# Geryyy/sspp

Hardware: AMD Instinct MI355X
Metric: candidate paths scored/sec (7-DoF, 128 waypts) at 1/2/4/8 MI355X; HBM %peak (higher is better)
Workload: dtype f64; 1 GPU; robocrane SamplingPathPlanner7 (block_green free joint), sigma 0.08; candidates_per_gpu=4096, waypoints=128, init_points=10, degree=3, dof=7, sampler=fp64, pair_order=hit, waypoint_order=hit, sampled_pairs=4, cylinder_box=False, capsule=False, scan=fp32-filtered, split=True, split_lost=0, split_handoffs=0, streams=4

## Files before the change

### include/sspp_hip.h

```cpp
#ifndef SSPP_HIP_H
#define SSPP_HIP_H
#include <stddef.h>
#include <stdint.h>

#ifdef __cplusplus
extern "C" {
#endif

#define SSPP_OK 0
#define SSPP_E_INVAL (-1)
#define SSPP_E_HIP (-2)
#define SSPP_E_SCENE (-3)
#define SSPP_E_NOMEM (-4)
#define SSPP_E_UNSUPPORTED (-5)
#define SSPP_E_IO (-6)
#define SSPP_E_INCOMPLETE (-7)

#define SSPP_GEOM_PLANE 0
#define SSPP_GEOM_SPHERE 2
#define SSPP_GEOM_CAPSULE 3
#define SSPP_GEOM_CYLINDER 5
#define SSPP_GEOM_BOX 6
#define SSPP_GEOM_MESH 7

// ... 111 lines not shown
                              double* d_vias_out , sspp_best* d_best,
                              void* stream);
int sspp_job_tsp_score_vias(sspp_job* job, const double* d_vias ,
                            int64_t first_id, int64_t B, double* d_L, double* d_Cnf,
                            double* d_Cwf, uint8_t* d_status, double* d_cost, sspp_best* d_best,
                            void* stream);
int sspp_job_info(const sspp_job* job, int* lanes_per_candidate, int* candidates_per_block,
                  int* block_threads, size_t* lds_bytes);
void sspp_job_free(sspp_job* job);

#define SSPP_OPT_SHAPE_NT 1
#define SSPP_OPT_SHAPE_G1 2
#define SSPP_OPT_ORDER 3
#define SSPP_OPT_TSP_FORM 4
#define SSPP_OPT_TSP_GENERIC 5
#define SSPP_OPT_SAMPLER 6
#define SSPP_OPT_LAST_NT 7
#define SSPP_OPT_LAST_G1 8
#define SSPP_OPT_WP_ORDER 9
#define SSPP_OPT_PREPASS_US 10
#define SSPP_OPT_NPAIRS 11
#define SSPP_OPT_CYLBOX 12
#define SSPP_OPT_F32 13
#define SSPP_OPT_LAST_F32 14
#define SSPP_OPT_CREATE_US 15
#define SSPP_OPT_PREPASS_STATE 16
#define SSPP_OPT_SPLIT 17
#define SSPP_OPT_LAST_SPLIT 18
#define SSPP_OPT_SPLIT_LINGER_US 20
#define SSPP_OPT_SPLIT_DROP 21
#define SSPP_OPT_SPLIT_HANDOFFS 22
#define SSPP_OPT_SPLIT_LOST 23
#define SSPP_OPT_CAPSULE 24
#define SSPP_OPT_TSP_REP 19
int sspp_job_set_option(sspp_job* job, int key, int64_t value);
int sspp_job_get_option(const sspp_job* job, int key, int64_t* value);

typedef struct sspp_ces sspp_ces;
typedef struct sspp_ces_config {
    int samples;
    int checks;
    int total_points;
    double w_collision, elite_fraction, inc, dec;
    double sigma_floor, var_beta, mean_lr, stddev_min, stddev_max;
    double z_min;
    double dist_z_min;
    double sigma0;
    const double* lo;
    const double* hi;
    double floor_z_min, floor_margin, floor_scale;
    uint64_t seed;
} sspp_ces_config;
typedef struct sspp_ces_info {
    int n_vias, n_slots, slots_per_rank, world, elite_capacity;
    int64_t iteration;
} sspp_ces_info;
typedef struct sspp_ces_state {
    int n_fixed;
    int n_candidates;
    int n_success, n_elite, has_best;
    int64_t best_slot;
    double best_cost;
    int64_t iteration;
} sspp_ces_state;
typedef struct sspp_ces_buffers {
    double *L, *C_nf, *C_wf, *cost;
// ... 78 lines not shown
```

### sspp_amd/_lib.py

```python
from __future__ import annotations

import ctypes as C
import os
import re

_HERE = os.path.dirname(os.path.abspath(__file__))
PRODUCT_LIB_PATH = os.path.join(_HERE, "lib", "libsspp_hip.so")
LIB_PATH = os.environ.get("SSPP_LIB_PATH") or PRODUCT_LIB_PATH
HEADER_PATH = os.path.join(os.path.dirname(_HERE), "include", "sspp_hip.h")

SSPP_OK = 0
SSPP_E_INCOMPLETE = -7
MODE_QPOS = 0
MODE_BODY = 1


class SsppError(RuntimeError):
    pass


class ModelView(C.Structure):
    _fields_ = [
        ("nbody", C.c_int), ("body_parent", C.POINTER(C.c_int32)),
        ("body_jnt_type", C.POINTER(C.c_int32)), ("body_qpos_adr", C.POINTER(C.c_int32)),
# ... 110 lines not shown
    "sspp_job_update_sspp": (C.c_int, [_vp, _d, C.c_double, _d, C.c_uint64, _vp]),
    "sspp_planner_create": (C.c_int, [_vp, _i, C.POINTER(_vp)]),
    "sspp_planner_plan": (C.c_int, [_vp, _d, _d, C.c_double, _d, _i, _i, _i, C.c_uint64, _i64, _d,
                                    C.POINTER(_i64), C.POINTER(_i64), _d, _d, C.POINTER(Best)]),
    "sspp_planner_score": (C.c_int, [_vp, _d, _i, _d, _i64, _i, _i, _i, _d, C.POINTER(C.c_uint8),
                                     C.POINTER(Best)]),
    "sspp_planner_free": (None, [_vp]),
    "sspp_planner_get_option": (C.c_int, [_vp, _i, C.POINTER(_i64)]),
    "sspp_ces_create": (C.c_int, [_vp, C.POINTER(CesConfig), _i, C.POINTER(_vp)]),
    "sspp_ces_get_info": (C.c_int, [_vp, C.POINTER(CesInfo)]),
    "sspp_ces_begin": (C.c_int, [_vp, _d, _d, _i, _vp]),
    "sspp_ces_eval": (C.c_int, [_vp, _i, _vp]),
    "sspp_ces_update": (C.c_int, [_vp, _vp]),
    "sspp_ces_plan": (C.c_int, [_vp, _d, _d, _i, _i, _vp]),
    "sspp_ces_plan_group": (C.c_int, [_vp, _i, _d, _d, _i, _i, _vp]),
    "sspp_ces_get_buffers": (C.c_int, [_vp, C.POINTER(CesBuffers)]),
    "sspp_ces_read": (C.c_int, [_vp, C.POINTER(CesState), _vp, _vp, _vp, _vp, _vp, _vp, _vp, _vp,
                                _vp, _vp]),
    "sspp_ces_set_state": (C.c_int, [_vp, _vp, _vp, _vp, _i]),
    "sspp_ces_pack": (C.c_int, [_vp, _i, _vp, _vp]),
    "sspp_ces_unpack": (C.c_int, [_vp, _vp, _vp]),
    "sspp_ces_free": (None, [_vp]),
    "sspp_job_set_option": (C.c_int, [_vp, _i, _i64]),
    "sspp_job_get_option": (C.c_int, [_vp, _i, C.POINTER(_i64)]),
    "sspp_ces_set_option": (C.c_int, [_vp, _i, _i64]),
}

OPT_SHAPE_NT, OPT_SHAPE_G1, OPT_ORDER, OPT_TSP_FORM, OPT_TSP_GENERIC = 1, 2, 3, 4, 5
OPT_SAMPLER, OPT_LAST_NT, OPT_LAST_G1, OPT_WP_ORDER, OPT_PREPASS_US, OPT_NPAIRS = 6, 7, 8, 9, 10, 11
OPT_CYLBOX, OPT_F32, OPT_LAST_F32, OPT_CREATE_US, OPT_PREPASS_STATE = 12, 13, 14, 15, 16
OPT_SPLIT, OPT_LAST_SPLIT, OPT_TSP_REP = 17, 18, 19
OPT_SPLIT_LINGER_US, OPT_SPLIT_DROP, OPT_SPLIT_HANDOFFS, OPT_SPLIT_LOST = 20, 21, 22, 23
OPT_CAPSULE = 24
OPT_CES_FUSED = 101


def declared_symbols(header=HEADER_PATH):
    txt = open(header).read()
    txt = re.sub(r"/\*.*?\*/", "", txt, flags=re.S)
    return sorted(set(re.findall(r"\b(sspp_[a-z_0-9]+)\s*\(", txt)))


_lib = None
build_warning = None


def check_revision(L, path, variant):
    from ._stamp import source_hash
    tree = source_hash()
    f = getattr(L, "sspp_build_id", None)
    built = None
    if f is not None:
        f.restype, f.argtypes = C.c_char_p, []
        built = (f() or b"").decode(errors="replace")
    if tree is None or built == tree:
        return None
    what = ("built from sources %s" % built) if built else "no source stamp (sspp_build_id)"
    msg = "%s: %s, but the tree's sources are %s" % (path, what, tree)
    if variant:
        raise SsppError("stale variant library " + msg +
                        " (rebuild it: bash tools/build_variant.sh NAME FLAGS)")
    import warnings
    warnings.warn("libsspp_hip.so does not match its sources: " + msg + " (run `make`)", RuntimeWarning)
    return msg


# ... 26 lines not shown
```

### sspp_amd/csrc/sspp_kern.h

```cpp
#pragma once
#include <hip/hip_runtime.h>

#include <algorithm>
#include <atomic>
#include <cstdlib>
#include <cmath>
#include <cstring>
#include <string>
#include <thread>
#include <vector>

#include "model.h"
#ifndef SSPP_TSP_REP_FORMS
#define SSPP_TSP_REP_FORMS (1 << 3)
#endif
#ifdef SSPP_TSP_STATS
__device__ unsigned long long g_tsp_stats[16];
#define TSP_STAT(i, c) do { const unsigned long long m_ = __ballot(c), a_ = __ballot(1);                  \
        if (__lane_id() == __builtin_ctzll(a_) && m_) atomicAdd(&g_tsp_stats[i], (unsigned long long)__popcll(m_)); } while (0)
#else
#define TSP_STAT(i, c) do { } while (0)
#endif
#ifdef SSPP_C2F_STATS
__device__ unsigned long long g_c2f_stats[16];
#define SSPP_CB_STAT(i) atomicAdd(&g_c2f_stats[i], 1ull)
#endif
#ifdef SSPP_WG_TIMING
__device__ unsigned long long g_wg_t[1 << 18];
__device__ unsigned long long g_wg_ph[8 << 16];
#define WG_PH(k) do { if (threadIdx.x == 0 && blockIdx.x < (1 << 16)) g_wg_ph[8 * blockIdx.x + (k)] = clock64(); } while (0)
__device__ unsigned long long g_p2_t[8 << 12];
__device__ unsigned long long g_p2_w[8 << 13];
#else
#define WG_PH(k) do { } while (0)
#endif
#include "sspp_device.h"
#include "sspp_filter.h"
#include "sspp_logtab.h"

using namespace sspd;

namespace sspk {

constexpr int kBlock = 256;
#ifndef SSPP_SCORE_WAVES_PER_EU
#define SSPP_SCORE_WAVES_PER_EU 4
#endif
constexpr int kMaxMovers = 2;
constexpr int kMaxSteps = 64;

constexpr int kTableCylBox = 1, kTableCapsule = 2;
__host__ __device__ inline int table_bits(int tg, int to) {
    return (((tg == 5 && to == 6) || (tg == 6 && to == 5)) ? kTableCylBox : 0) |
           (sspd::pair_has_capsule(tg, to) ? kTableCapsule : 0);
}

struct KScene {
    int npairs;
    int onegeom;
    int static_block;
    double static_cost;
    int cylbox;
    int upright;
    int cbup;
};
// ... 748 lines not shown
#define SSPP_QUEUE_ACQUIRE() do { } while (0)
#endif
#ifndef SSPP_SPLIT_PRIO
#define SSPP_SPLIT_PRIO 1
#endif
#ifndef SSPP_PRIO_ALL
#define SSPP_PRIO_ALL 0
#endif
#ifndef SSPP_SPLIT_PRIO_CONSUMER
#define SSPP_SPLIT_PRIO_CONSUMER 0
#endif
#ifndef SSPP_QUEUE_WAITERS
#define SSPP_QUEUE_WAITERS 4
#endif
#ifndef SSPP_LINGER_SLEEP
#define SSPP_LINGER_SLEEP 16
#endif
constexpr int kSurvShards = 64;
struct SurvShard {
    unsigned count;
    unsigned taken;
    unsigned pushed;
    unsigned served;
    unsigned pad[28];
};
struct SurvQ {
    SurvShard shard[kSurvShards];
    unsigned nlist;
    unsigned lost;
    unsigned norphan;
    unsigned pad1;
    unsigned long long handoffs;
    unsigned long long lost_total;
    unsigned pad2[24];
    unsigned arrive_sh[8][32];
    unsigned arrive_top[32];
    unsigned long long bestbits[kMaxSteps];
    unsigned count_feas[kMaxSteps];
};
__host__ __device__ inline unsigned long long surv_word(int step, long long lc, bool defer) {
    return (1ull << 63) | ((unsigned long long)defer << 62) | ((unsigned long long)(unsigned)step << 32) |
           (unsigned long long)(unsigned)lc;
}
struct SurvBest {
    unsigned long long bits, id, step, pad;
};
struct SurvPtrs {
    SurvQ* hdr;
    unsigned long long* rec;
    double* ctrl;
    float* ctrl32;
    SurvBest* res;
    unsigned* orphan;
#ifdef SSPP_DEBUG_PROGRESS
    unsigned* beacon;
#endif
    long long cap;
    int shard_cap;
};

struct SsppC2F {
    KScene sc;
    int has_scene;
    int sampler;
    int p, n, W;
    double sigma;
    unsigned long long seed;
    long long first_id, B;
    int g1, cpw, cpb;
    int npts, n1;
    int lpc;
    int nblk_step;
    long long step_stride;
    int arc_all;
    int r0, r1;
    int nt;
    int lds;
    int ctrl_feas;
    int f32;
    float feps, fplim;
    int split;
    int nsteps;
    int drop_orphans;
    unsigned long long linger;
};

#ifdef SSPP_C2F_STATS
#define C2F_STAT(i, v) do { const unsigned long long v_ = (v); if ((threadIdx.x & 63) == 0 && v_) atomicAdd(&g_c2f_stats[i], v_); } while (0)
#else
#define C2F_STAT(i, v) do { } while (0)
#endif

__device__ __forceinline__ int crow(int mine, int fix, int r0, int r1, int j, int D) {
    return (j >= r0 && j < r1) ? mine + (j - r0) * D : fix + j * D;
}
template <int D, int P>
__device__ __forceinline__ void eval_split(const double* sm, int mine, int fix, int r0, int r1,
                                           const double (&Nr)[P + 1], int span, double* q) {
    int o[P + 1];
#pragma unroll
    for (int r = 0; r <= P; ++r) o[r] = crow(mine, fix, r0, r1, span - P + r, D);
#pragma unroll
    for (int d = 0; d < D; ++d) {
        double acc = Nr[0] * sm[o[0] + d];
#pragma unroll
// ... 402 lines not shown
#pragma unroll
                for (int d = 0; d < D; ++d) qa[d] = __shfl_up(qb[d], 1, 64);
                if (lane == 0) eval_split_g<D, P>(smem, o_own, o_fix, r0, r1, atab + jj * P1, aspan[jj], qa);
                if (jc < nch) acc = acc + dist_nd<D>(qa, qb);
            }
            acc = wave_sum(acc);
            if (lane == 0) s_vsum[vw] = acc;
        }
        SSPP_BEACON(23, slot, 0);
        __syncthreads();
        total = s_vsum[0];
        for (int w = 1; w < nvw; ++w) total = total + s_vsum[w];
    }
    if (tid == 0) {
        const long long c = (long long)step * a.B + lc;
        arc[c] = total;
        feasible[c] = (unsigned char)feas;
        if (with_best) {
            if (feas && total < INFINITY) {
                const unsigned long long bits = (unsigned long long)__double_as_longlong(total);
                const unsigned long long seen =
                    __hip_atomic_fetch_min(q.hdr->bestbits + step, bits, __ATOMIC_RELAXED, __HIP_MEMORY_SCOPE_AGENT);
                if (bits <= seen) {
                    const unsigned k = __hip_atomic_fetch_add(&q.hdr->nlist, 1u, __ATOMIC_RELAXED, __HIP_MEMORY_SCOPE_AGENT);
                    __hip_atomic_store(&q.res[k].bits, bits, __ATOMIC_RELAXED, __HIP_MEMORY_SCOPE_AGENT);
                    __hip_atomic_store(&q.res[k].id, (unsigned long long)(a.first_id + step * a.step_stride + lc),
                                       __ATOMIC_RELAXED, __HIP_MEMORY_SCOPE_AGENT);
                    __hip_atomic_store(&q.res[k].step, (unsigned long long)step, __ATOMIC_RELAXED, __HIP_MEMORY_SCOPE_AGENT);
                }
            }
            if (feas) __hip_atomic_fetch_add(q.hdr->count_feas + step, 1u, __ATOMIC_RELAXED, __HIP_MEMORY_SCOPE_AGENT);
        }
#ifdef SSPP_WG_TIMING
        unsigned long long* t = g_p2_w + 8 * (slot & ((8u << 10) - 1u));
        t[0] = w_t0; t[1] = wall_clock64(); t[2] = w_np; t[3] = w_nf; t[4] = feas;
        t[5] = c1 - c0; t[6] = clock64() - c1; t[7] = blockIdx.x;
#endif
    }
    (void)slot;
    SSPP_BEACON(24, slot, 0);
    __syncthreads();
}

#ifndef SSPP_C2F_WAVES_PER_EU
#define SSPP_C2F_WAVES_PER_EU 5
#endif
#ifndef SSPP_C2F_WAVES_PER_EU_WIDE
#define SSPP_C2F_WAVES_PER_EU_WIDE 4
#endif
#ifndef SSPP_ABLATE
#define SSPP_ABLATE 0
#endif
template <int D, int NM, int P, bool ONEGEOM, int NT, bool CBX, bool SPLIT = false>
#ifndef SSPP_C2F_FIVE_MAX
#define SSPP_C2F_FIVE_MAX 128
#endif
#ifndef SSPP_C2F_GP_NT
#define SSPP_C2F_GP_NT 256
#endif
__global__ __launch_bounds__(NT, (NT <= SSPP_C2F_FIVE_MAX && ONEGEOM) ? SSPP_C2F_WAVES_PER_EU : SSPP_C2F_WAVES_PER_EU_WIDE) void k_sspp_c2f(
    SsppC2F a, SceneT T, const double* __restrict__ otab, const float* __restrict__ otab32,
    const int* __restrict__ ospan,
    const double* __restrict__ atab, const int* __restrict__ aspan,
    const double* __restrict__ init_ctrl, const double* __restrict__ limits,
    const double* __restrict__ ctrl_in, double* __restrict__ ctrl_out, double* __restrict__ arc,
    unsigned char* __restrict__ feasible, BlockBest* __restrict__ part, ArgminSync* sync, sspp_best* best,
    SurvPtrs q) {
    extern __shared__ __attribute__((aligned(16))) double smem[];
    constexpr int P1 = P + 1;
// ... 102 lines not shown
    {
        const bool valid = in_grp && g < nvalid;
        bool ghit = false, dfr = false;
        if (collide_on) {
            const bool live = valid && l < a.n1 && !a.sc.static_block && !(ABL & 16);
            const int own = o_own + (valid ? g : 0) * nrd;
            if (f32) {
                float q32[D];
                eval_split32<D, P>(s_f32, own, o_fix, r0, r1, N32_p1, span_p1, q32);
                unsigned long long amb;
                ghit = scan_pairs32<D, NM, ONEGEOM>(q32, live, ~0ull, ~0ull, gbits, a.sc, TT, a.feps, a.fplim, amb);
                const bool need = live && !ghit && amb != 0ull;
                C2F_STAT(11, __popcll(__ballot(need)));
                if (__ballot(need) != 0ull) {
                    double q[D];
                    eval_split_g<D, P>(smem, own, o_fix, r0, r1, otab + row_p1 * P1, span_p1, q);
                    ghit = scan_pairs<D, NM, ONEGEOM, CBX ? 1 : 0>(q, need, amb, wave_or64(need ? amb : 0ull), gbits, nullptr,
                                                      a.sc, TT, dfr) || ghit;
                }
            } else {
                double q[D];
                eval_split_g<D, P>(smem, own, o_fix, r0, r1, otab + row_p1 * P1, span_p1, q);
                ghit = scan_pairs<D, NM, ONEGEOM, CBX ? 1 : 0>(q, live, ~0ull, ~0ull, gbits, nullptr, a.sc, TT, dfr);
            }
        }
        const bool gdef = (__ballot(dfr) & gbits) != 0ull;
        if (in_grp && l == 0 && g < cpb) {
            s_feas[g] = valid && !ghit && !(collide_on && a.sc.static_block);
            s_defer[g] = gdef;
        }
    }
    __syncthreads();
    WG_PH(3);
    if constexpr ((SPLIT || SSPP_PRIO_ALL) && SSPP_SPLIT_PRIO) __builtin_amdgcn_s_setprio(SSPP_SPLIT_PRIO_CONSUMER);
    if constexpr (SPLIT) {
        static_assert(NM == 1 && ONEGEOM && !CBX, "split launches: single-geom movers without cylinder-box pairs");
        int tid_s = threadIdx.x;
        asm volatile("" : "+v"(tid_s));
        const int tid = tid_s;
        SSPP_BEACON(3, 0, 0);
        SSPP_BEACON_T(1);
        if (tid < 64) {
            const bool f = tid < nvalid && s_feas[tid] != 0;
            const unsigned long long m = __ballot(f);
            unsigned base = 0;
            if (tid == 0 && m)
                base = __hip_atomic_fetch_add(&q.hdr->shard[blockIdx.x % kSurvShards].count, (unsigned)__popcll(m),
                                              __ATOMIC_RELAXED, __HIP_MEMORY_SCOPE_AGENT);
            base = (unsigned)__shfl((int)base, 0, 64) + (unsigned)((blockIdx.x % kSurvShards) * q.shard_cap);
            if (tid < cpb) s_surv[tid] = f ? (int)(base + __popcll(m & ((1ull << tid) - 1ull))) : -1;
        }
        __syncthreads();
        for (int e = tid; e < nvalid * nrd; e += NT) {
            const int sl = e / nrd, r = e - sl * nrd, slot = s_surv[sl];
            if (slot >= 0) {
                const long long o = (long long)slot * nrd + r;
                __hip_atomic_store((unsigned long long*)q.ctrl + o,
                                   (unsigned long long)__double_as_longlong(smem[o_own + sl * nrd + r]),
                                   __ATOMIC_RELAXED, __HIP_MEMORY_SCOPE_AGENT);
                __hip_atomic_store((unsigned*)q.ctrl32 + o, __float_as_uint(s_f32[o_own + sl * nrd + r]),
                                   __ATOMIC_RELAXED, __HIP_MEMORY_SCOPE_AGENT);
            }
        }
        asm volatile("s_waitcnt vmcnt(0)" ::: "memory");
        __syncthreads();
        if (tid < nvalid) {
            const int slot = s_surv[tid];
            if (slot >= 0) {
                __hip_atomic_store(q.rec + slot, surv_word(step, cand0 + tid, s_defer[tid] != 0), SSPP_QUEUE_RELEASE_ORDER,
                                   __HIP_MEMORY_SCOPE_AGENT);
            } else {
                arc[tid + cand0] = INFINITY;
                feasible[tid + cand0] = 0;
            }
        }
        asm volatile("s_waitcnt vmcnt(0)" ::: "memory");
        __syncthreads();
        if (tid == 0)
            __hip_atomic_fetch_add(&q.hdr->shard[blockIdx.x % kSurvShards].pushed, 1u, __ATOMIC_RELAXED,
                                   __HIP_MEMORY_SCOPE_AGENT);
        SSPP_BEACON(4, __popcll(__ballot(tid < nvalid && s_surv[tid] >= 0)), __smid());
        SSPP_BEACON_T(2);
        const unsigned nb_all = gridDim.x, shs = blockIdx.x % kSurvShards;
        const unsigned nwg_s = (nb_all - shs + kSurvShards - 1) / kSurvShards;
        SurvShard* const sh = q.hdr->shard + shs;
        int* s_ctl = s_surv;
        int* s_last = s_surv + cpb;
        bool last = false;
        unsigned ko = 0, no = 0;
        unsigned handed = 0;
#ifdef SSPP_DEBUG_PROGRESS
        unsigned nfin = 0;
#endif
        for (;;) {
            if (tid == 0) {
                unsigned t = ~0u;
                unsigned long long w = 0ull;
                if (!last) {
                    const unsigned tk0 = __hip_atomic_load(&sh->taken, __ATOMIC_RELAXED, __HIP_MEMORY_SCOPE_AGENT);
                    const unsigned ct0 = __hip_atomic_load(&sh->count, __ATOMIC_RELAXED, __HIP_MEMORY_SCOPE_AGENT);
                    if ((int)(tk0 - ct0) < SSPP_QUEUE_WAITERS) {
                        t = __hip_atomic_fetch_add(&sh->taken, 1u, __ATOMIC_RELAXED, __HIP_MEMORY_SCOPE_AGENT);
                        SSPP_BEACON(5, t, ct0);
                        const unsigned long long w0 = wall_clock64();
                        for (;;) {
                            if (t < __hip_atomic_load(&sh->count, __ATOMIC_RELAXED, __HIP_MEMORY_SCOPE_AGENT)) break;
                            if (__hip_atomic_load(&sh->pushed, __ATOMIC_RELAXED, __HIP_MEMORY_SCOPE_AGENT) >= nwg_s &&
                                __hip_atomic_load(&sh->count, __ATOMIC_RELAXED, __HIP_MEMORY_SCOPE_AGENT) <= t) {
                                t = ~0u;
                                break;
                            }
                            if (wall_clock64() - w0 >= a.linger) {
                                const unsigned k = __hip_atomic_fetch_add(&q.hdr->norphan, 1u, __ATOMIC_RELAXED,
                                                                          __HIP_MEMORY_SCOPE_AGENT);
                                __hip_atomic_store(q.orphan + k, t + shs * (unsigned)q.shard_cap, __ATOMIC_RELAXED,
                                                   __HIP_MEMORY_SCOPE_AGENT);
                                handed = 1;
                                t = ~0u;
                                break;
                            }
                            __builtin_amdgcn_s_sleep(SSPP_LINGER_SLEEP);
                        }
                    }
                    if (t != ~0u) {
                        t += shs * (unsigned)q.shard_cap;
                        SSPP_BEACON(6, t, 0);
                        const unsigned long long w1 = wall_clock64();
                        while ((w = __hip_atomic_load(q.rec + t, __ATOMIC_RELAXED, __HIP_MEMORY_SCOPE_AGENT)) == 0ull) {
                            if (wall_clock64() - w1 >= a.linger) break;
                            __builtin_amdgcn_s_sleep(1);
                        }
// ... 47 lines not shown
                const unsigned nblk = gridDim.x;
                const int shd = blockIdx.x & 7, nsh = nblk < 8 ? (int)nblk : 8;
                if (tid == 0) {
                    asm volatile("s_waitcnt vmcnt(0)" ::: "memory");
                    const unsigned shard_n = (nblk - shd + 7) >> 3;
                    const unsigned prev = __hip_atomic_fetch_add(&q.hdr->arrive_sh[shd][0], 1u + (handed << 16),
                                                                 __ATOMIC_RELAXED, __HIP_MEMORY_SCOPE_AGENT);
                    int lst = 0;
                    if ((prev & 0xFFFFu) == shard_n - 1) {
                        const unsigned sho = (prev >> 16) + handed;
                        const unsigned pt = __hip_atomic_fetch_add(&q.hdr->arrive_top[0], 1u + (sho << 16),
                                                                   __ATOMIC_RELAXED, __HIP_MEMORY_SCOPE_AGENT);
                        lst = (pt & 0xFFFFu) == (unsigned)nsh - 1;
                        if (lst) {
                            SSPP_QUEUE_ACQUIRE();
                            no = (pt >> 16) + sho;
                        }
                    }
                    s_last[0] = lst;
                    s_last[1] = (int)no;
                }
                __syncthreads();
                const int lst = __builtin_amdgcn_readfirstlane(s_last[0]);
                SSPP_BEACON(9 + lst, no, 0);
                if (lst) SSPP_BEACON_E(0);
                if (!lst) return;
                if (__builtin_amdgcn_readfirstlane(s_last[1]) == 0) break;
                last = true;
                continue;
            }
            const unsigned long long w = ((unsigned long long)(unsigned)__builtin_amdgcn_readfirstlane(s_ctl[2]) << 32) |
                                         (unsigned)__builtin_amdgcn_readfirstlane(s_ctl[3]);
            SSPP_BEACON(7, t, (unsigned)w);
            surv_load_rows<NT>(q, t, nrd, smem, s_f32, o_own);
            __syncthreads();
            surv_finish<D, NM, P, ONEGEOM, NT>(a, TT, otab, otab32, ospan, atab, aspan, smem, s_f32, o_fix, o_own,
                                               s_ctl, s_vsum, w, t, arc_base, feas_base, best_base != nullptr, q);
            if (tid == 0)
                __hip_atomic_fetch_add(&q.hdr->shard[t / (unsigned)q.shard_cap].served, 1u, __ATOMIC_RELAXED,
                                       __HIP_MEMORY_SCOPE_AGENT);
#ifdef SSPP_DEBUG_PROGRESS
            if (tid == 0 && q.beacon) q.beacon[8 * blockIdx.x + 3] = ++nfin;
#endif
        }
#ifdef SSPP_WG_TIMING
        const unsigned long long t_ep = wall_clock64();
#endif
        asm volatile("s_waitcnt vmcnt(0)" ::: "memory");
        __syncthreads();
        SSPP_BEACON(12, no, 0);
        SSPP_BEACON_E(1);
        int tid_e = threadIdx.x;
        asm volatile("" : "+v"(tid_e));
        const int tid_ep = tid_e;
        unsigned long long* s_bits = (unsigned long long*)smem;
        unsigned long long* s_id = s_bits + kMaxSteps;
        unsigned* s_cnt = (unsigned*)(s_id + kMaxSteps);
        unsigned* s_lost = s_cnt + kMaxSteps;
        const int nsteps = a.nsteps;
        const unsigned nl = __hip_atomic_load(&q.hdr->nlist, __ATOMIC_RELAXED, __HIP_MEMORY_SCOPE_AGENT);
        unsigned c_sh = 0, sv_sh = 0;
        if (tid_ep < kSurvShards) {
            c_sh = __hip_atomic_load(&q.hdr->shard[tid_ep].count, __ATOMIC_RELAXED, __HIP_MEMORY_SCOPE_AGENT);
            sv_sh = __hip_atomic_load(&q.hdr->shard[tid_ep].served, __ATOMIC_RELAXED, __HIP_MEMORY_SCOPE_AGENT);
        }
        unsigned long long rb = 0ull, rid = 0ull, rst = 0ull;
        if (best_base) {
            rb = __hip_atomic_load(&q.res[tid_ep].bits, __ATOMIC_RELAXED, __HIP_MEMORY_SCOPE_AGENT);
            rid = __hip_atomic_load(&q.res[tid_ep].id, __ATOMIC_RELAXED, __HIP_MEMORY_SCOPE_AGENT);
            rst = __hip_atomic_load(&q.res[tid_ep].step, __ATOMIC_RELAXED, __HIP_MEMORY_SCOPE_AGENT);
        }
        for (int e = tid_ep; e < nsteps; e += NT) {
            s_bits[e] = __hip_atomic_load(q.hdr->bestbits + e, __ATOMIC_RELAXED, __HIP_MEMORY_SCOPE_AGENT);
            s_cnt[e] = __hip_atomic_load(q.hdr->count_feas + e, __ATOMIC_RELAXED, __HIP_MEMORY_SCOPE_AGENT);
            s_id[e] = ~0ull;
        }
        const unsigned short_sh = c_sh > sv_sh ? c_sh - sv_sh : 0u;
        if (tid_ep < 64) {
            const unsigned tot = (unsigned)wave_sum_u32((int)short_sh);
            if (tid_ep == 0) s_lost[0] = tot;
        }
        __syncthreads();
        const unsigned lost = (unsigned)__builtin_amdgcn_readfirstlane((int)s_lost[0]);
        SSPP_BEACON_E(2);
        if (short_sh)
            for (unsigned e = 0; e < c_sh; ++e)
                __hip_atomic_store(q.rec + (unsigned)tid_ep * (unsigned)q.shard_cap + e, 0ull, __ATOMIC_RELAXED,
                                   __HIP_MEMORY_SCOPE_AGENT);
        if (tid_ep == 0) {
            if (lost) __hip_atomic_fetch_add(&q.hdr->lost_total, (unsigned long long)lost, __ATOMIC_RELAXED,
                                             __HIP_MEMORY_SCOPE_AGENT);
            if (no) __hip_atomic_fetch_add(&q.hdr->handoffs, (unsigned long long)no, __ATOMIC_RELAXED,
                                           __HIP_MEMORY_SCOPE_AGENT);
        }
        if (best_base) {
            if ((unsigned)tid_ep < nl && rb == s_bits[rst]) atomicMin(s_id + rst, rid);
            for (unsigned i = tid_ep + NT; i < nl; i += NT) {
                const unsigned long long bits = __hip_atomic_load(&q.res[i].bits, __ATOMIC_RELAXED, __HIP_MEMORY_SCOPE_AGENT);
                const unsigned long long id = __hip_atomic_load(&q.res[i].id, __ATOMIC_RELAXED, __HIP_MEMORY_SCOPE_AGENT);
                const int st = (int)__hip_atomic_load(&q.res[i].step, __ATOMIC_RELAXED, __HIP_MEMORY_SCOPE_AGENT);
                if (bits == s_bits[st]) atomicMin(s_id + st, id);
            }
        }
        __syncthreads();
        SSPP_BEACON_E(3);
        for (int e = tid_ep; e < nsteps; e += NT) {
            if (best_base) {
                const bool has = s_id[e] != ~0ull;
                best_base[e].cost = has ? __longlong_as_double((long long)s_bits[e]) : INFINITY;
                best_base[e].index = has ? (long long)s_id[e] : -1;
                best_base[e].count = s_cnt[e];
                best_base[e].reserved = lost;
            }
// ... 905 lines not shown
    double* d_pp_term = nullptr;
    unsigned* d_pp_arrive = nullptr;
    int64_t pp_cap = 0;
    unsigned char* h_pin = nullptr;
    size_t h_pin_bytes = 0;
    hipEvent_t upd_ev = nullptr;
    bool upd_pending = false;
    double start[4], end[4], lo[4], hi[4];
    double z_min = 0, w_col = 1, floor_z_min = 0, floor_margin = 0.01, floor_scale = 10;
    std::thread prepass_thread;
    std::atomic<int> prepass_state{0};
    std::vector<int> pre_wps;
    std::vector<DPair> pre_pairs, pre_pairs_s;
    double pre_ms = 0.0;
    int pre_gen = 0;
    int tables_gen = 0;
    hipStream_t pre_stream = nullptr;
    hipEvent_t pre_ev = nullptr;
    unsigned long long* d_hits = nullptr;
    unsigned long long* h_hits = nullptr;
    DPair* d_census_pairs = nullptr;
    std::vector<void*> retired;
    double create_ms = 0.0;
    int opt_split = 1;
    int last_split = 0;
    SurvQ* d_sq_hdr = nullptr;
    unsigned long long* d_sq_rec = nullptr;
    double* d_sq_ctrl = nullptr;
    float* d_sq_ctrl32 = nullptr;
    SurvBest* d_sq_res = nullptr;
    unsigned* d_sq_orphan = nullptr;
    int opt_linger_us = 10000;
    int opt_split_drop = 0;
    unsigned* dbg_beacon = nullptr;
    long long sq_cap = 0;
    int sq_nrd = 0;
};


namespace sspk {

inline KScene kscene(const sspp_scene* s, bool tsp, bool generic = false) {
    KScene k{};
    if (!s) return k;
    k.npairs = (int)s->pairs.size();
    k.onegeom = 1;
    for (const DPair& p : s->pairs) k.onegeom &= (p.gm == s->pairs[0].gm);
    k.static_block = (!tsp && s->count_static && s->static_contacts > 0) ? 1 : 0;
    k.static_cost = tsp ? s->static_cost : 0.0;
    k.upright = (tsp && !generic) ? 1 : 0;
    k.cbup = k.upright;
    for (const DPair& p : s->pairs) {
        const DGeom& g = s->geoms[p.gm];
        const int tg = g.type;
        k.cylbox |= table_bits(tg, p.otype);
        if (sspd::pair_has_capsule(tg, p.otype)) k.upright = k.cbup = 0;
        if (tg == 6 && p.otype == 6)
            k.upright &= (!g.relrot || sspd::upright3(g.mat)) && sspd::upright3(p.omat);
        if (tg == 5 && p.otype == 6)
            k.cbup &= (!g.relrot || sspd::cyl_vertical(g.mat)) && sspd::upright3(p.omat);
        if (tg == 6 && p.otype == 5)
            k.cbup &= (!g.relrot || sspd::upright3(g.mat)) && sspd::cyl_vertical(p.omat);
    }
    return k;
}

// ... 258 lines not shown
```

### sspp_amd/csrc/sspp_kernels.hip

```cpp
#include "sspp_kern.h"

#include <chrono>
#include <random>

using namespace sspk;

#ifndef SSPP_SINGLE_TU
namespace sspk {
SSPK_ENTRY_DECL(extern, 1, 2)
SSPK_ENTRY_DECL(extern, 1, 3)
SSPK_ENTRY_DECL(extern, 2, 2)
SSPK_ENTRY_DECL(extern, 2, 3)
SSPK_ENTRY_DECL(extern, 3, 2)
SSPK_ENTRY_DECL(extern, 3, 3)
SSPK_ENTRY_DECL(extern, 4, 2)
SSPK_ENTRY_DECL(extern, 4, 3)
SSPK_ENTRY_DECL(extern, 6, 2)
SSPK_ENTRY_DECL(extern, 6, 3)
SSPK_ENTRY_DECL(extern, 7, 2)
SSPK_ENTRY_DECL(extern, 7, 3)
SSPK_ENTRY_DECL(extern, 9, 2)
SSPK_ENTRY_DECL(extern, 9, 3)
SSPK_TSP_DECL(extern)
}
// ... 967 lines not shown
    c.first_id = first_id; c.B = B;
    c.g1 = g1; c.cpw = cpw; c.cpb = cpb; c.npts = j->W + 1; c.n1 = std::min(g1, j->W + 1);
    c.lpc = lanes_for(j->W - 1);
    c.nblk_step = nblk;
    c.step_stride = step_stride;
    c.arc_all = j->arc_all;
    c.r0 = r0; c.r1 = r1;
    c.nt = nt; c.lds = (int)lds;
    c.ctrl_feas = j->ctrl_feas;
    const double feps = j->f32 && c.has_scene ? f32_eps(j->scene, d_ctrl ? j->h_pairs : j->h_pairs_s) : 0.0;
    c.f32 = feps > 0.0 ? 1 : 0;
    c.feps = (float)feps;
    c.fplim = kF32PosLimit;
    j->last_nt = nt; j->last_g1 = g1; j->last_f32 = c.f32;
    c.nsteps = steps;
    c.split = j->opt_split && (int64_t)steps * B >= kSplitMinCands && !d_ctrl && !d_ctrl_out && !j->arc_all &&
              (int64_t)nblk * steps < 65536 &&
              c.has_scene && c.sc.npairs > 0 && !c.sc.static_block && j->nm == 1 && c.sc.onegeom && !c.sc.cylbox &&
              cpb >= 3;
    SurvPtrs q{};
    int split_used = 0;
    if (c.split) {
        const int nb_all = nblk * steps;
        const int shard_cap = ((nb_all + kSurvShards - 1) / kSurvShards) * cpb;
        int rc = survq_reserve(j, (int64_t)shard_cap * kSurvShards, nrd);
        if (rc) return rc;
        q = SurvPtrs{j->d_sq_hdr, j->d_sq_rec, j->d_sq_ctrl, j->d_sq_ctrl32, j->d_sq_res, j->d_sq_orphan,
#ifdef SSPP_DEBUG_PROGRESS
                     j->dbg_beacon,
#endif
                     j->sq_cap, shard_cap};
        c.linger = (unsigned long long)j->opt_linger_us * 100ull;
        c.drop_orphans = j->opt_split_drop;
        c.lds = std::max(c.lds, (int)(20 * kMaxSteps + 16));
    }
    SsppPtrs o{d_ctrl, d_ctrl_out, d_arc, d_feasible, d_best, q, &split_used};
    const int nb = nblk * steps;
    hipError_t e = hipErrorInvalidValue;
    switch (j->D) {
#ifndef SSPP_DEV_ONLY
        case 1: e = entry_c2f<1>(c, j, o, nb, st); break;
        case 2: e = entry_c2f<2>(c, j, o, nb, st); break;
        case 3: e = entry_c2f<3>(c, j, o, nb, st); break;
        case 4: e = entry_c2f<4>(c, j, o, nb, st); break;
        case 6: e = entry_c2f<6>(c, j, o, nb, st); break;
        case 9: e = entry_c2f<9>(c, j, o, nb, st); break;
#endif
        case 7: e = entry_c2f<7>(c, j, o, nb, st); break;
    }
    j->last_split = split_used;
    if (e != hipSuccess) return hip_fail(e, "k_sspp_c2f launch");
    return SSPP_OK;
}

extern "C" int sspp_job_sample_score(sspp_job* j, int64_t first_id, int64_t B, double* d_arc,
                          uint8_t* d_feasible, double* d_ctrl_out, sspp_best* d_best, void* stream) {
    return run_sspp(j, nullptr, first_id, B, d_arc, d_feasible, d_ctrl_out, d_best, stream);
}

extern "C" int sspp_job_update_sspp(sspp_job* j, const double* init_ctrl, double sigma,
                                    const double* limits, uint64_t seed, void* stream) {
    sspp::clear_error();
    if (!j || j->kind != 0 || !init_ctrl || !limits) return sspp::set_error(SSPP_E_INVAL, "sspp_job_update_sspp: bad argument");
    const size_t nd = (size_t)j->n * j->D;
    hipStream_t st = (hipStream_t)stream;
    j->seed = seed;
// ... 45 lines not shown
    switch (key) {
        case SSPP_OPT_SHAPE_NT:
            if (j->kind != 0 || !(value == 0 || value == 64 || value == 128 || value == 256))
                return sspp::set_error(SSPP_E_INVAL, "SSPP_OPT_SHAPE_NT: 0, 64, 128 or 256");
            j->opt_nt = (int)value;
            return SSPP_OK;
        case SSPP_OPT_SHAPE_G1:
            if (j->kind != 0 || value < 0 || value > 64)
                return sspp::set_error(SSPP_E_INVAL, "SSPP_OPT_SHAPE_G1: 0 (per launch) or 1..64");
            j->opt_g1 = (int)value;
            return SSPP_OK;
        case SSPP_OPT_ORDER: {
            if (j->kind != 0 || value < 0 || value > 2) return sspp::set_error(SSPP_E_INVAL, "SSPP_OPT_ORDER: 0, 1 or 2");
            prepass_drop(j);
            HIPCHK(hipDeviceSynchronize());
            const size_t nd = (size_t)j->n * j->D;
            return set_job_tables(j, j->h_stage.data(), j->sigma, j->h_stage.data() + nd, (int)value, true, nullptr);
        }
        case SSPP_OPT_TSP_FORM:
            if (j->kind != 1 || value < -1 || value > 4) return sspp::set_error(SSPP_E_INVAL, "SSPP_OPT_TSP_FORM: -1..4");
            j->tsp_form = (int)value;
            return SSPP_OK;
        case SSPP_OPT_TSP_GENERIC:
            if (j->kind != 1) return sspp::set_error(SSPP_E_INVAL, "SSPP_OPT_TSP_GENERIC: TaskSpacePlanner jobs only");
            j->tsp_generic = value ? 1 : 0;
            return SSPP_OK;
        case SSPP_OPT_F32:
            if (j->kind != 0 || value < 0 || value > 1) return sspp::set_error(SSPP_E_INVAL, "SSPP_OPT_F32: 0 or 1");
            j->f32 = (int)value;
            return SSPP_OK;
        case SSPP_OPT_SPLIT:
            if (j->kind != 0 || value < 0 || value > 1) return sspp::set_error(SSPP_E_INVAL, "SSPP_OPT_SPLIT: 0 or 1");
            j->opt_split = (int)value;
            return SSPP_OK;
        case SSPP_OPT_SPLIT_LINGER_US:
            if (j->kind != 0 || value < 0 || value > 1000000)
                return sspp::set_error(SSPP_E_INVAL, "SSPP_OPT_SPLIT_LINGER_US: 0..1000000");
            j->opt_linger_us = (int)value;
            return SSPP_OK;
        case SSPP_OPT_SPLIT_DROP:
            if (j->kind != 0 || value < 0 || value > 1) return sspp::set_error(SSPP_E_INVAL, "SSPP_OPT_SPLIT_DROP: 0 or 1");
            j->opt_split_drop = (int)value;
            return SSPP_OK;
#ifdef SSPP_DEBUG_PROGRESS
        case 900:
            j->dbg_beacon = (unsigned*)(uintptr_t)value;
            return SSPP_OK;
#endif
        case SSPP_OPT_TSP_REP:
            if (j->kind != 1 || value < -1 || value == 0 || value > 16)
                return sspp::set_error(SSPP_E_INVAL, "SSPP_OPT_TSP_REP: -1 or 1..16");
            j->tsp_rep = (int)value;
            return SSPP_OK;
    }
    return sspp::set_error(SSPP_E_INVAL, "unknown or read-only option");
}

extern "C" int sspp_job_get_option(const sspp_job* j, int key, int64_t* value) {
    if (!j || !value) return sspp::set_error(SSPP_E_INVAL, "null argument");
    switch (key) {
        case SSPP_OPT_SHAPE_NT: *value = j->opt_nt; return SSPP_OK;
        case SSPP_OPT_SHAPE_G1: *value = j->opt_g1; return SSPP_OK;
        case SSPP_OPT_ORDER: *value = j->pair_order; return SSPP_OK;
        case SSPP_OPT_TSP_FORM: *value = j->kind == 1 ? j->last_form : -1; return SSPP_OK;
        case SSPP_OPT_TSP_GENERIC: *value = j->tsp_generic; return SSPP_OK;
        case SSPP_OPT_SAMPLER: *value = j->sampler; return SSPP_OK;
        case SSPP_OPT_LAST_NT: *value = j->last_nt; return SSPP_OK;
        case SSPP_OPT_LAST_G1: *value = j->last_g1; return SSPP_OK;
        case SSPP_OPT_WP_ORDER: *value = j->wp_order; return SSPP_OK;
        case SSPP_OPT_PREPASS_US: *value = (int64_t)(j->prepass_ms * 1e3); return SSPP_OK;
        case SSPP_OPT_NPAIRS: *value = j->np_samp; return SSPP_OK;
        case SSPP_OPT_CYLBOX: *value = (j->cb_samp & sspk::kTableCylBox) != 0; return SSPP_OK;
        case SSPP_OPT_CAPSULE: *value = (j->cb_samp & sspk::kTableCapsule) != 0; return SSPP_OK;
        case SSPP_OPT_F32: *value = j->f32; return SSPP_OK;
        case SSPP_OPT_LAST_F32: *value = j->last_f32; return SSPP_OK;
        case SSPP_OPT_CREATE_US: *value = (int64_t)(j->create_ms * 1e3); return SSPP_OK;
        case SSPP_OPT_SPLIT: *value = j->opt_split; return SSPP_OK;
        case SSPP_OPT_LAST_SPLIT: *value = j->last_split; return SSPP_OK;
        case SSPP_OPT_SPLIT_LINGER_US: *value = j->opt_linger_us; return SSPP_OK;
        case SSPP_OPT_SPLIT_DROP: *value = j->opt_split_drop; return SSPP_OK;
        case SSPP_OPT_SPLIT_HANDOFFS:
        case SSPP_OPT_SPLIT_LOST: {
            *value = 0;
            if (!j->d_sq_hdr) return SSPP_OK;
            SurvQ h;
            HIPCHK(hipDeviceSynchronize());
            HIPCHK(hipMemcpy(&h, j->d_sq_hdr, sizeof(SurvQ), hipMemcpyDeviceToHost));
            *value = (int64_t)(key == SSPP_OPT_SPLIT_HANDOFFS ? h.handoffs : h.lost_total);
            return SSPP_OK;
        }
        case SSPP_OPT_TSP_REP: *value = j->kind == 1 ? j->last_rep : 0; return SSPP_OK;
        case SSPP_OPT_PREPASS_STATE: *value = j->prepass_state.load(std::memory_order_acquire); return SSPP_OK;
    }
    return sspp::set_error(SSPP_E_INVAL, "unknown option");
}

extern "C" int sspp_job_create_tsp(const sspp_scene* scene, const sspp_tsp_args* a, int64_t max_batch,
                        sspp_job** out) {
    sspp::clear_error();
    if (!scene || !a || !out || !a->start || !a->end || !a->lo || !a->hi)
        return sspp::set_error(SSPP_E_INVAL, "sspp_job_create_tsp: null argument");
    if (scene->mode != SSPP_MODE_BODY) return sspp::set_error(SSPP_E_INVAL, "scene must be bound to a body");
    const int K = a->n_vias, cp = a->check_points, n = K + 2;
    if (K < 0 || K > 60) return sspp::set_error(SSPP_E_INVAL, "n_vias out of range");
    if (K > 0 && (!a->mean || !a->sigma)) return sspp::set_error(SSPP_E_INVAL, "null mean/sigma");
    if (cp < 1 || cp > 1 << 20) return sspp::set_error(SSPP_E_INVAL, "check_points must be >= 1");
    if (max_batch < 1) return sspp::set_error(SSPP_E_INVAL, "max_batch must be >= 1");
    if (n < 3) return sspp::set_error(SSPP_E_INVAL, "degree-2 interpolation needs >= 3 points");
    auto* j = new sspp_job();
    j->kind = 1; j->scene = scene; j->D = 4; j->p = 2; j->n = n; j->K = K; j->cp = cp;
    j->nknots = n + 3; j->seed = a->seed; j->max_batch = max_batch; j->nm = 1;
    for (int i = 0; i < 4; ++i) { j->start[i] = a->start[i]; j->end[i] = a->end[i]; j->lo[i] = a->lo[i]; j->hi[i] = a->hi[i]; }
    j->z_min = a->z_min; j->w_col = a->w_collision;
    j->floor_z_min = a->floor_z_min; j->floor_margin = a->floor_margin; j->floor_scale = a->floor_scale;
    j->lpc = lanes_for(cp);
    j->cpb = kBlock / j->lpc;
    j->lds = sizeof(double) * ((size_t)2 * j->cpb * n * 4 + 3 * (kBlock / 64) + 4) + sizeof(int) * j->cpb;
    if (j->lds > 160 * 1024) { delete j; return sspp::set_error(SSPP_E_UNSUPPORTED, "problem too large for LDS"); }
    std::vector<double> u(n), knots(n + 3), Minv((size_t)2 * n * n + n);
    for (int i = 0; i < n; ++i) u[i] = (double)i / (n - 1);
    if (sspp::qr_program(u.data(), n, 2, knots.data(), Minv.data()) != 0) {
// ... 434 lines not shown
```

### sspp_amd/runtime.py

```python
from __future__ import annotations

import ctypes as C
import math

import numpy as np

from . import _lib
from ._lib import (Best, CesBuffers, CesConfig, CesInfo, CesState, ModelView, SceneInfo,
                   SsppArgs, TspArgs, check, lib)

DEFAULT_SEED = 0x5EED
SAMPLER_FP64, SAMPLER_FP32 = 0, 1


def _dptr(a):
    return a.ctypes.data_as(C.POINTER(C.c_double))


def _f64(x, n=None):
    a = np.ascontiguousarray(np.asarray(x, dtype=np.float64).reshape(-1))
    if n is not None and a.size != n:
        raise ValueError("expected %d values, got %d" % (n, a.size))
    return a

# ... 202 lines not shown

    def alloc(self, B, device="cuda", with_ctrl=False):
        torch = _torch()
        out = dict(arc=torch.empty(B, dtype=torch.float64, device=device),
                   feasible=torch.empty(B, dtype=torch.uint8, device=device),
                   best=best_tensor(device))
        if with_ctrl:
            out["ctrl"] = torch.empty((B, self.n, self.D), dtype=torch.float64, device=device)
        return out

    def sample_score(self, first_id, B, arc, feasible, best, ctrl_out=None, stream=None):
        check(lib().sspp_job_sample_score(self._h, int(first_id), int(B), _ptr(arc), _ptr(feasible),
                                          _ptr(ctrl_out), _ptr(best), _stream(stream)),
              "sample_score")

    def score_ctrl(self, ctrl, first_id, arc, feasible, best, stream=None):
        B = ctrl.shape[0]
        check(lib().sspp_job_score_ctrl(self._h, _ptr(ctrl), int(first_id), int(B), _ptr(arc),
                                        _ptr(feasible), _ptr(best), _stream(stream)), "score_ctrl")

    def set_shape(self, nt=0, g1=0):
        self.set_option(_lib.OPT_SHAPE_NT, nt)
        self.set_option(_lib.OPT_SHAPE_G1, g1)

    def config(self):
        g = self.get_option
        return dict(sampler="fp32" if g(_lib.OPT_SAMPLER) else "fp64",
                    shape="%dx%d" % (g(_lib.OPT_LAST_NT), g(_lib.OPT_LAST_G1)),
                    pair_order={0: "scene", 1: "gap", 2: "hit"}[g(_lib.OPT_ORDER)],
                    waypoint_order={0: "bisection", 2: "hit"}[g(_lib.OPT_WP_ORDER)],
                    prepass_ms=g(_lib.OPT_PREPASS_US) / 1e3, sampled_pairs=g(_lib.OPT_NPAIRS),
                    cylinder_box=bool(g(_lib.OPT_CYLBOX)), capsule=bool(g(_lib.OPT_CAPSULE)),
                    scan="fp32-filtered" if g(_lib.OPT_LAST_F32) else "fp64",
                    split=bool(g(_lib.OPT_LAST_SPLIT)))


class TspJob(_Job):

    def __init__(self, scene, start, end, n_vias, check_points, mean=None, sigma=None,
                 lo=(-2, -2, -2, -2), hi=(2, 2, 2, 2), z_min=0.0, w_collision=1.0,
                 seed=DEFAULT_SEED, max_batch=4096, floor=(0.0, 0.01, 10.0)):
        K = int(n_vias)
        self.start, self.end = _f64(start, 4), _f64(end, 4)
        self.mean = _f64(mean if mean is not None else np.zeros((max(K, 1), 4)))
        self.sigma = _f64(sigma if sigma is not None else np.zeros((max(K, 1), 4)))
        self.lo, self.hi = _f64(lo, 4), _f64(hi, 4)
        self.K, self.cp, self.max_batch = K, int(check_points), int(max_batch)
        a = TspArgs(start=_dptr(self.start), end=_dptr(self.end), n_vias=K, check_points=self.cp,
                    w_collision=float(w_collision), mean=_dptr(self.mean), sigma=_dptr(self.sigma),
                    lo=_dptr(self.lo), hi=_dptr(self.hi), z_min=float(z_min),
                    seed=int(seed) & (2 ** 64 - 1), floor_z_min=float(floor[0]),
                    floor_margin=float(floor[1]), floor_scale=float(floor[2]))
        h = C.c_void_p()
        check(lib().sspp_job_create_tsp(scene.handle, C.byref(a), self.max_batch, C.byref(h)),
              "job create (tsp)")
        self._h = h
        self.scene = scene

    def alloc(self, B, device="cuda", with_vias=False):
        torch = _torch()
        f = lambda: torch.empty(B, dtype=torch.float64, device=device)
        out = dict(L=f(), Cnf=f(), Cwf=f(), cost=f(),
                   status=torch.empty(B, dtype=torch.uint8, device=device),
                   best=best_tensor(device))
        if with_vias:
            out["vias"] = torch.empty((B, max(self.K, 1), 4), dtype=torch.float64, device=device)
        return out
# ... 198 lines not shown
```

Baseline: 3.451 billion candidate paths/s.

## Keep first feasible survivor local to producer workgroup instead of queueing it

In the split scoring kernel, each producer workgroup now keeps its first feasible candidate in its own LDS and finishes it itself, and pushes only the remaining survivors to the global survivor queue. When no other survivors exist, the global ctrl/ctrl32 stores and their waitcnt/barriers are skipped entirely. This is meant to cut global queue traffic, atomics and handoff latency. It adds a local-slot encoding (kSurvLocal) and a queued-count statistic, and it changes how work is balanced across workgroups. The new path is on by default through an option.

Result: slower. 3.403 billion candidate paths/s (-1.4%).

```diff
diff --git a/include/sspp_hip.h b/include/sspp_hip.h
--- a/include/sspp_hip.h
+++ b/include/sspp_hip.h
@@ -167,6 +167,8 @@
 #define SSPP_OPT_SPLIT_HANDOFFS 22
 #define SSPP_OPT_SPLIT_LOST 23
 #define SSPP_OPT_CAPSULE 24
+#define SSPP_OPT_SPLIT_LOCAL 25
+#define SSPP_OPT_SPLIT_QUEUED 26
 #define SSPP_OPT_TSP_REP 19
 int sspp_job_set_option(sspp_job* job, int key, int64_t value);
 int sspp_job_get_option(const sspp_job* job, int key, int64_t* value);
diff --git a/sspp_amd/_lib.py b/sspp_amd/_lib.py
--- a/sspp_amd/_lib.py
+++ b/sspp_amd/_lib.py
@@ -166,6 +166,7 @@
 OPT_SPLIT, OPT_LAST_SPLIT, OPT_TSP_REP = 17, 18, 19
 OPT_SPLIT_LINGER_US, OPT_SPLIT_DROP, OPT_SPLIT_HANDOFFS, OPT_SPLIT_LOST = 20, 21, 22, 23
 OPT_CAPSULE = 24
+OPT_SPLIT_LOCAL, OPT_SPLIT_QUEUED = 25, 26
 OPT_CES_FUSED = 101
 
 
diff --git a/sspp_amd/csrc/sspp_kern.h b/sspp_amd/csrc/sspp_kern.h
--- a/sspp_amd/csrc/sspp_kern.h
+++ b/sspp_amd/csrc/sspp_kern.h
@@ -31,6 +31,7 @@
 #define WG_PH(k) do { if (threadIdx.x == 0 && blockIdx.x < (1 << 16)) g_wg_ph[8 * blockIdx.x + (k)] = clock64(); } while (0)
 __device__ unsigned long long g_p2_t[8 << 12];
 __device__ unsigned long long g_p2_w[8 << 13];
+__device__ unsigned g_p2_n;
 #else
 #define WG_PH(k) do { } while (0)
 #endif
@@ -845,7 +846,8 @@
     unsigned pad1;
     unsigned long long handoffs;
     unsigned long long lost_total;
-    unsigned pad2[24];
+    unsigned long long queued_total;
+    unsigned pad2[22];
     unsigned arrive_sh[8][32];
     unsigned arrive_top[32];
     unsigned long long bestbits[kMaxSteps];
@@ -855,6 +857,7 @@
     return (1ull << 63) | ((unsigned long long)defer << 62) | ((unsigned long long)(unsigned)step << 32) |
            (unsigned long long)(unsigned)lc;
 }
+constexpr unsigned kSurvLocal = 0xFFFFFF00u;
 struct SurvBest {
     unsigned long long bits, id, step, pad;
 };
@@ -884,6 +887,7 @@
     int npts, n1;
     int lpc;
     int nblk_step;
+    int split_local;
     long long step_stride;
     int arc_all;
     int r0, r1;
@@ -1352,9 +1356,10 @@
             if (feas) __hip_atomic_fetch_add(q.hdr->count_feas + step, 1u, __ATOMIC_RELAXED, __HIP_MEMORY_SCOPE_AGENT);
         }
 #ifdef SSPP_WG_TIMING
-        unsigned long long* t = g_p2_w + 8 * (slot & ((8u << 10) - 1u));
+        unsigned long long* t = g_p2_w + 8 * (atomicAdd(&g_p2_n, 1u) & ((8u << 10) - 1u));
         t[0] = w_t0; t[1] = wall_clock64(); t[2] = w_np; t[3] = w_nf; t[4] = feas;
-        t[5] = c1 - c0; t[6] = clock64() - c1; t[7] = blockIdx.x;
+        t[5] = c1 - c0; t[6] = clock64() - c1; t[7] = blockIdx.x | ((unsigned long long)(step * a.nblk_step + lc / a.cpb) << 20) |
+               ((unsigned long long)(slot >= 0xFFFFFF00u) << 40);
 #endif
     }
     (void)slot;
@@ -1523,6 +1528,9 @@
     }
     __syncthreads();
     WG_PH(3);
+#ifdef SSPP_WG_TIMING
+    if (SPLIT && threadIdx.x == 0 && blockIdx.x < (1 << 16)) g_wg_ph[8 * blockIdx.x + 7] = wall_clock64();
+#endif
     if constexpr ((SPLIT || SSPP_PRIO_ALL) && SSPP_SPLIT_PRIO) __builtin_amdgcn_s_setprio(SSPP_SPLIT_PRIO_CONSUMER);
     if constexpr (SPLIT) {
         static_assert(NM == 1 && ONEGEOM && !CBX, "split launches: single-geom movers without cylinder-box pairs");
@@ -1531,46 +1539,76 @@
         const int tid = tid_s;
         SSPP_BEACON(3, 0, 0);
         SSPP_BEACON_T(1);
+        int* s_loc = (int*)s_mask;
         if (tid < 64) {
             const bool f = tid < nvalid && s_feas[tid] != 0;
             const unsigned long long m = __ballot(f);
+            const unsigned long long mq = a.split_local ? m & (m - 1ull) : m;
+            const bool fq = ((mq >> tid) & 1ull) != 0ull;
             unsigned base = 0;
-            if (tid == 0 && m)
-                base = __hip_atomic_fetch_add(&q.hdr->shard[blockIdx.x % kSurvShards].count, (unsigned)__popcll(m),
+            if (tid == 0 && mq)
+                base = __hip_atomic_fetch_add(&q.hdr->shard[blockIdx.x % kSurvShards].count, (unsigned)__popcll(mq),
                                               __ATOMIC_RELAXED, __HIP_MEMORY_SCOPE_AGENT);
             base = (unsigned)__shfl((int)base, 0, 64) + (unsigned)((blockIdx.x % kSurvShards) * q.shard_cap);
-            if (tid < cpb) s_surv[tid] = f ? (int)(base + __popcll(m & ((1ull << tid) - 1ull))) : -1;
+            if (tid < cpb) s_surv[tid] = fq ? (int)(base + __popcll(mq & ((1ull << tid) - 1ull))) : -1;
+            if (tid == 0) {
+                s_loc[1] = __popcll(mq);
+                if (m == mq) s_loc[0] = -1;
+                s_loc[4] = m != mq;
+            }
+            if (f && !fq) {
+                const unsigned long long w = surv_word(step, cand0 + tid, s_defer[tid] != 0);
+                s_loc[0] = tid;
+                s_loc[2] = (int)(unsigned)(w >> 32);
+                s_loc[3] = (int)(unsigned)w;
+            }
         }
         __syncthreads();
-        for (int e = tid; e < nvalid * nrd; e += NT) {
-            const int sl = e / nrd, r = e - sl * nrd, slot = s_surv[sl];
-            if (slot >= 0) {
-                const long long o = (long long)slot * nrd + r;
-                __hip_atomic_store((unsigned long long*)q.ctrl + o,
-                                   (unsigned long long)__double_as_longlong(smem[o_own + sl * nrd + r]),
-                                   __ATOMIC_RELAXED, __HIP_MEMORY_SCOPE_AGENT);
-                __hip_atomic_store((unsigned*)q.ctrl32 + o, __float_as_uint(s_f32[o_own + sl * nrd + r]),
-                                   __ATOMIC_RELAXED, __HIP_MEMORY_SCOPE_AGENT);
-            }
-        }
-        asm volatile("s_waitcnt vmcnt(0)" ::: "memory");
-        __syncthreads();
+        const int nq = __builtin_amdgcn_readfirstlane(s_loc[1]);
+        const int kept = __builtin_amdgcn_readfirstlane(s_loc[0]);
+        const bool qpath = nq > 0 || !a.split_local;
+        if (qpath) {
+            for (int e = tid; e < nvalid * nrd; e += NT) {
+                const int sl = e / nrd, r = e - sl * nrd, slot = s_surv[sl];
+                if (slot >= 0) {
+                    const long long o = (long long)slot * nrd + r;
+                    __hip_atomic_store((unsigned long long*)q.ctrl + o,
+                                       (unsigned long long)__double_as_longlong(smem[o_own + sl * nrd + r]),
+                                       __ATOMIC_RELAXED, __HIP_MEMORY_SCOPE_AGENT);
+                    __hip_atomic_store((unsigned*)q.ctrl32 + o, __float_as_uint(s_f32[o_own + sl * nrd + r]),
+                                       __ATOMIC_RELAXED, __HIP_MEMORY_SCOPE_AGENT);
+                }
+            }
+            asm volatile("s_waitcnt vmcnt(0)" ::: "memory");
+            __syncthreads();
+        }
         if (tid < nvalid) {
-            const int slot = s_surv[tid];
+            const int slot = qpath ? s_surv[tid] : -1;
             if (slot >= 0) {
                 __hip_atomic_store(q.rec + slot, surv_word(step, cand0 + tid, s_defer[tid] != 0), SSPP_QUEUE_RELEASE_ORDER,
                                    __HIP_MEMORY_SCOPE_AGENT);
-            } else {
+            } else if (tid != kept) {
                 arc[tid + cand0] = INFINITY;
                 feasible[tid + cand0] = 0;
             }
         }
-        asm volatile("s_waitcnt vmcnt(0)" ::: "memory");
-        __syncthreads();
+        if (qpath) {
+            asm volatile("s_waitcnt vmcnt(0)" ::: "memory");
+            __syncthreads();
+        }
         if (tid == 0)
             __hip_atomic_fetch_add(&q.hdr->shard[blockIdx.x % kSurvShards].pushed, 1u, __ATOMIC_RELAXED,
                                    __HIP_MEMORY_SCOPE_AGENT);
-        SSPP_BEACON(4, __popcll(__ballot(tid < nvalid && s_surv[tid] >= 0)), __smid());
+        SSPP_BEACON(4, nq, __smid());
+#ifdef SSPP_WG_TIMING
+        {
+            const unsigned wq = (unsigned)nq;
+            if (tid == 0 && blockIdx.x < (1 << 16)) {
+                g_wg_ph[8 * blockIdx.x + 5] = wq;
+                g_wg_ph[8 * blockIdx.x + 6] = wall_clock64();
+            }
+        }
+#endif
         SSPP_BEACON_T(2);
         const unsigned nb_all = gridDim.x, shs = blockIdx.x % kSurvShards;
         const unsigned nwg_s = (nb_all - shs + kSurvShards - 1) / kSurvShards;
@@ -1587,7 +1625,11 @@
             if (tid == 0) {
                 unsigned t = ~0u;
                 unsigned long long w = 0ull;
-                if (!last) {
+                if (s_loc[4]) {
+                    s_loc[4] = 0;
+                    t = kSurvLocal | (unsigned)s_loc[0];
+                    w = ((unsigned long long)(unsigned)s_loc[2] << 32) | (unsigned)s_loc[3];
+                } else if (!last) {
                     const unsigned tk0 = __hip_atomic_load(&sh->taken, __ATOMIC_RELAXED, __HIP_MEMORY_SCOPE_AGENT);
                     const unsigned ct0 = __hip_atomic_load(&sh->count, __ATOMIC_RELAXED, __HIP_MEMORY_SCOPE_AGENT);
                     if ((int)(tk0 - ct0) < SSPP_QUEUE_WAITERS) {
@@ -1701,11 +1743,13 @@
             const unsigned long long w = ((unsigned long long)(unsigned)__builtin_amdgcn_readfirstlane(s_ctl[2]) << 32) |
                                          (unsigned)__builtin_amdgcn_readfirstlane(s_ctl[3]);
             SSPP_BEACON(7, t, (unsigned)w);
-            surv_load_rows<NT>(q, t, nrd, smem, s_f32, o_own);
+            const bool loc = t >= kSurvLocal;
+            const int o_rows = o_own + (loc ? (int)(t & 0xFFu) * nrd : 0);
+            if (!loc) surv_load_rows<NT>(q, t, nrd, smem, s_f32, o_own);
             __syncthreads();
-            surv_finish<D, NM, P, ONEGEOM, NT>(a, TT, otab, otab32, ospan, atab, aspan, smem, s_f32, o_fix, o_own,
+            surv_finish<D, NM, P, ONEGEOM, NT>(a, TT, otab, otab32, ospan, atab, aspan, smem, s_f32, o_fix, o_rows,
                                                s_ctl, s_vsum, w, t, arc_base, feas_base, best_base != nullptr, q);
-            if (tid == 0)
+            if (tid == 0 && !loc)
                 __hip_atomic_fetch_add(&q.hdr->shard[t / (unsigned)q.shard_cap].served, 1u, __ATOMIC_RELAXED,
                                        __HIP_MEMORY_SCOPE_AGENT);
 #ifdef SSPP_DEBUG_PROGRESS
@@ -1747,7 +1791,12 @@
         const unsigned short_sh = c_sh > sv_sh ? c_sh - sv_sh : 0u;
         if (tid_ep < 64) {
             const unsigned tot = (unsigned)wave_sum_u32((int)short_sh);
-            if (tid_ep == 0) s_lost[0] = tot;
+            const unsigned totq = (unsigned)wave_sum_u32((int)c_sh);
+            if (tid_ep == 0) {
+                s_lost[0] = tot;
+                if (totq) __hip_atomic_fetch_add(&q.hdr->queued_total, (unsigned long long)totq, __ATOMIC_RELAXED,
+                                                 __HIP_MEMORY_SCOPE_AGENT);
+            }
         }
         __syncthreads();
         const unsigned lost = (unsigned)__builtin_amdgcn_readfirstlane((int)s_lost[0]);
@@ -2719,6 +2768,7 @@
     unsigned* d_sq_orphan = nullptr;
     int opt_linger_us = 10000;
     int opt_split_drop = 0;
+    int opt_split_local = 1;
     unsigned* dbg_beacon = nullptr;
     long long sq_cap = 0;
     int sq_nrd = 0;
diff --git a/sspp_amd/csrc/sspp_kernels.hip b/sspp_amd/csrc/sspp_kernels.hip
--- a/sspp_amd/csrc/sspp_kernels.hip
+++ b/sspp_amd/csrc/sspp_kernels.hip
@@ -1023,6 +1023,7 @@
                      j->sq_cap, shard_cap};
         c.linger = (unsigned long long)j->opt_linger_us * 100ull;
         c.drop_orphans = j->opt_split_drop;
+        c.split_local = j->opt_split_local;
         c.lds = std::max(c.lds, (int)(20 * kMaxSteps + 16));
     }
     SsppPtrs o{d_ctrl, d_ctrl_out, d_arc, d_feasible, d_best, q, &split_used};
@@ -1134,6 +1135,10 @@
         case SSPP_OPT_SPLIT:
             if (j->kind != 0 || value < 0 || value > 1) return sspp::set_error(SSPP_E_INVAL, "SSPP_OPT_SPLIT: 0 or 1");
             j->opt_split = (int)value;
+            return SSPP_OK;
+        case SSPP_OPT_SPLIT_LOCAL:
+            if (j->kind != 0 || value < 0 || value > 1) return sspp::set_error(SSPP_E_INVAL, "SSPP_OPT_SPLIT_LOCAL: 0 or 1");
+            j->opt_split_local = (int)value;
             return SSPP_OK;
         case SSPP_OPT_SPLIT_LINGER_US:
             if (j->kind != 0 || value < 0 || value > 1000000)
@@ -1181,14 +1186,17 @@
         case SSPP_OPT_LAST_SPLIT: *value = j->last_split; return SSPP_OK;
         case SSPP_OPT_SPLIT_LINGER_US: *value = j->opt_linger_us; return SSPP_OK;
         case SSPP_OPT_SPLIT_DROP: *value = j->opt_split_drop; return SSPP_OK;
+        case SSPP_OPT_SPLIT_LOCAL: *value = j->opt_split_local; return SSPP_OK;
         case SSPP_OPT_SPLIT_HANDOFFS:
+        case SSPP_OPT_SPLIT_QUEUED:
         case SSPP_OPT_SPLIT_LOST: {
             *value = 0;
             if (!j->d_sq_hdr) return SSPP_OK;
             SurvQ h;
             HIPCHK(hipDeviceSynchronize());
             HIPCHK(hipMemcpy(&h, j->d_sq_hdr, sizeof(SurvQ), hipMemcpyDeviceToHost));
-            *value = (int64_t)(key == SSPP_OPT_SPLIT_HANDOFFS ? h.handoffs : h.lost_total);
+            *value = (int64_t)(key == SSPP_OPT_SPLIT_HANDOFFS ? h.handoffs
+                               : key == SSPP_OPT_SPLIT_QUEUED ? h.queued_total : h.lost_total);
             return SSPP_OK;
         }
         case SSPP_OPT_TSP_REP: *value = j->kind == 1 ? j->last_rep : 0; return SSPP_OK;
diff --git a/sspp_amd/runtime.py b/sspp_amd/runtime.py
--- a/sspp_amd/runtime.py
+++ b/sspp_amd/runtime.py
@@ -258,7 +258,7 @@
                     prepass_ms=g(_lib.OPT_PREPASS_US) / 1e3, sampled_pairs=g(_lib.OPT_NPAIRS),
                     cylinder_box=bool(g(_lib.OPT_CYLBOX)), capsule=bool(g(_lib.OPT_CAPSULE)),
                     scan="fp32-filtered" if g(_lib.OPT_LAST_F32) else "fp64",
-                    split=bool(g(_lib.OPT_LAST_SPLIT)))
+                    split=bool(g(_lib.OPT_LAST_SPLIT)), split_local=bool(g(_lib.OPT_SPLIT_LOCAL)))
 
 
 class TspJob(_Job):
```
